# NeLy-EPFL/DeepFly3D

Hardware: AMD Instinct MI355X
Metric: frames/sec (7-view 2D->3D) (higher is better)
Workload: dtype f32; 1 GPU; BASELINE configs[1]: 2176 frames x 7 views 256x512x3 per GPU, 2-stack hourglass fp32, arg-max + 38-joint layout + fp64 DLT; frames_per_gpu=2176, parallelism=frame-sharded x1, one packed gather, collective_executed=False

## Files before the change

### deepfly3d_amd/csrc/hg_launch.h

```cpp
#pragma once
#include "hg_plan.h"

namespace {

inline int cu_count() {
    static int cached[64] = {0};
    int dev = 0;
    if (hipGetDevice(&dev) != hipSuccess || dev < 0 || dev >= 64) return 256;
    if (cached[dev] == 0) {
        int n = 0;
        cached[dev] = hipDeviceGetAttribute(&n, hipDeviceAttributeMultiprocessorCount, dev) == hipSuccess && n > 0 ? n : 256;
    }
    return cached[dev];
}

inline bool first_use_on_this_device(unsigned& mask) {
    int dev = 0;
    if (hipGetDevice(&dev) != hipSuccess || dev < 0 || dev > 31) return true;
    const bool first = !(mask & (1u << dev));
    mask |= 1u << dev;
    return first;
}

hipEvent_t get_event(df3d_hg* h) {
// ... 15 lines not shown
    ScopedTimer(df3d_hg* h_, hipStream_t s_, const std::string& name, const Work& w) : h(h_), s(s_), on(h_->prof.profiling) {
        if (!on) return;
        t = {get_event(h), get_event(h), h->prof.kernel_class(name), w};
        if (w.flops_executed < 0.0) t.w.flops_executed = w.flops;
        (void)hipEventRecord(t.a, s);
    }
    ~ScopedTimer() {
        if (!on) return;
        (void)hipEventRecord(t.b, s);
        h->prof.timed.push_back(t);
    }
};

template <typename T> struct TypeName;
template <> struct TypeName<float> { static constexpr const char* value = "float"; };
template <> struct TypeName<__hip_bfloat16> { static constexpr const char* value = "__hip_bfloat16"; };
template <> struct TypeName<_Float16> { static constexpr const char* value = "_Float16"; };
template <> struct TypeName<F32S> { static constexpr const char* value = "hgk::F32S"; };
template <typename T> using StorageT = std::conditional_t<std::is_same<T, F32S>::value, float, T>;

inline std::string targ(bool v) { return v ? "true" : "false"; }
inline std::string targ(int v) { return std::to_string(v); }
inline std::string targ(const char* v) { return v; }
template <typename... A>
std::string kname(const char* kernel, A... args) {
    std::string s = kernel;
    const char* sep = "<";
    ((s += sep, s += targ(args), sep = ", "), ...);
    return sizeof...(A) ? s + ">" : s;
}

template <auto KERNEL, typename... A>
int launch_kernel(df3d_hg* h, const std::string& name, const Work& w, dim3 grid, int threads, int lds_bytes, hipStream_t s, const A&... args) {
    ScopedTimer tm(h, s, name, w);
    static unsigned attr_done = 0;
    if (lds_bytes > 0 && first_use_on_this_device(attr_done))
        DF3D_HIP(hipFuncSetAttribute(reinterpret_cast<const void*>(KERNEL), hipFuncAttributeMaxDynamicSharedMemorySize, lds_bytes));
    hipLaunchKernelGGL(KERNEL, grid, dim3(threads), lds_bytes, s, args...);
    DF3D_LAUNCH_CHECK();
    return DF3D_OK;
}

template <typename T, int TAPS, int BN, int RB>
int launch_conv_t(df3d_hg* h, const ConvArgs& a, const Work& w, hipStream_t s) {
    const dim3 grid((unsigned)((a.M + BM - 1) / BM), (unsigned)(a.cout / BN));
    return launch_kernel<conv_mfma_kernel<T, TAPS, BN, RB>>(h, kname("conv_mfma_kernel", TypeName<T>::value, TAPS, BN, RB), w, grid, 256,
                                                            2 * (BM + BN) * (RB + 16), s, a);
}

template <typename T, int TAPS, int BN>
int launch_conv_rb(df3d_hg* h, const ConvArgs& a, int rb, const Work& w, hipStream_t s) {
    if (rb == 128) return launch_conv_t<T, TAPS, BN, 128>(h, a, w, s);
    return launch_conv_t<T, TAPS, BN, 64>(h, a, w, s);
}

template <typename T>
int launch_conv(df3d_hg* h, const ConvArgs& a, int taps, int rb, const Work& w, hipStream_t s) {
    int bn = (a.cout % 128 == 0) ? 128 : (a.cout % 64 == 0 ? 64 : 32);
    const long long wgs128 = ((a.M + BM - 1) / BM) * (a.cout / bn);
    if (bn == 128 && wgs128 < 2LL * cu_count()) bn = taps == 1 ? 32 : 64;
    if (taps == 1) {
        if (bn == 128) return launch_conv_rb<T, 1, 128>(h, a, rb, w, s);
        if (bn == 64) return launch_conv_rb<T, 1, 64>(h, a, rb, w, s);
        return launch_conv_rb<T, 1, 32>(h, a, rb, w, s);
    }
    if (bn == 128) return launch_conv_rb<T, 9, 128>(h, a, rb, w, s);
    if (bn == 64) return launch_conv_rb<T, 9, 64>(h, a, rb, w, s);
    df3d::set_error("3x3 convolution with cout %d unsupported", a.cout);
    return DF3D_EINVAL;
}

template <typename T, bool LAST>
int launch_head(df3d_hg* h, const HeadArgs& a, const Work& w, hipStream_t s) {
    return launch_kernel<head_kernel<T, LAST>>(h, kname("head_kernel", TypeName<T>::value, LAST), w, dim3((unsigned)((a.M + 127) / 128)), 256,
                                               HeadCfg<T, LAST>::LDS_BYTES, s, a);
}

struct BtLaunch {
    double px, m1;
    int tiles;
    bool pool_only;
};
inline double bt_flops(double px, int cin, int pl, bool conv1, bool ds, double taps3 = 9.0) {
    return 2.0 * px * ((conv1 ? (double)cin * pl : 0.0) + taps3 * pl * pl + 2.0 * pl * pl + (ds ? 2.0 * cin * pl : 0.0));
}
inline double bt_bytes(double px, int eb, int cin, int pl, bool t1, bool pool_only) {
    return px * eb * (cin + (t1 ? pl : 0) + (pool_only ? 0.5 * pl : 2.0 * pl));
}

template <typename T, int CIN, int PL, bool DS, bool UP = false, bool ADD2 = false>
int launch_bottleneck_t(df3d_hg* h, const BottleneckArgs& a, const BtLaunch& b, hipStream_t s) {
    return launch_kernel<bottleneck_kernel<T, CIN, PL, DS, UP, ADD2>>(
        h, kname("bottleneck_kernel", TypeName<T>::value, CIN, PL, DS, UP, ADD2),
        Work{bt_flops(b.px, CIN, PL, true, DS), bt_bytes(b.px, sizeof(T), CIN, PL, false, false), b.m1}, dim3(b.tiles), 256,
        BtCfg<T, CIN, PL, DS>::LDS_BYTES, s, a);
}

template <typename F>
int with_up_add2(const void* in2, const void* add2, F&& f) {
    if (in2) return f(std::true_type{}, std::false_type{});
    if (add2) return f(std::false_type{}, std::true_type{});
    return f(std::false_type{}, std::false_type{});
}

template <typename T>
int launch_l1_lp(df3d_hg* h, const BtL1Args& a, const BtLaunch& b, hipStream_t s) {
    const int tiles = a.V * (a.H / L1_TH) * (a.W / BT_TW);
    return launch_kernel<bottleneck_l1_kernel<T>>(h, kname("bottleneck_l1_kernel", TypeName<T>::value),
                                                  Work{bt_flops(b.px, 64, 64, true, true), bt_bytes(b.px, sizeof(T), 64, 64, false, b.pool_only), b.m1},
                                                  dim3(std::min(tiles, cu_count())), L1_WAVES * 64, L1_LDS_BYTES, s, a);
}

template <typename T, bool UP, int CIN, bool ADD2, int MODE>
int launch_ring_lp_(df3d_hg* h, const BtRingArgs& r, const BtLaunch& b, int lds_bytes, hipStream_t s) {
    return launch_kernel<bottleneck_ring_kernel<T, UP, CIN, ADD2, MODE>>(
        h, kname("bottleneck_ring_kernel", TypeName<T>::value, UP, CIN, ADD2, MODE),
        Work{bt_flops(b.px, CIN, 128, true, CIN == 128), bt_bytes(b.px, sizeof(T), CIN, 128, false, false), b.m1}, dim3(b.tiles), 256, lds_bytes, s, r);
}
template <typename T, bool UP, int CIN, bool ADD2 = false>
int launch_ring_lp(df3d_hg* h, const BtRingArgs& r, const BtLaunch& b, int lds_bytes, hipStream_t s) {
    return !r.w2d    ? launch_ring_lp_<T, UP, CIN, ADD2, 0>(h, r, b, lds_bytes, s)
           : h->ring2 ? launch_ring_lp_<T, UP, CIN, ADD2, 2>(h, r, b, lds_bytes, s)
                      : launch_ring_lp_<T, UP, CIN, ADD2, 1>(h, r, b, lds_bytes, s);
}

template <typename T, bool UP, bool ADD2, bool TAIL>
int launch_ring_f32(df3d_hg* h, const BtRingArgs& r, const BtLaunch& b, int lds_bytes, hipStream_t s) {
    return launch_kernel<bottleneck_ring_f32_kernel<UP, ADD2, TAIL, T>>(
        h, kname("bottleneck_ring_f32_kernel", UP, ADD2, TAIL, TypeName<T>::value),
        Work{bt_flops(b.px, 256, 128, !TAIL, false), bt_bytes(b.px, 4, 256, 128, TAIL, false), b.m1}, dim3(b.tiles), 256, lds_bytes, s, r);
}

inline int ring_lds_bytes() {
    int lds_bytes = BR_LDS_BYTES;
#ifdef DF3D_BT_TIMING
    if (const char* e = getenv("BR_LDS")) lds_bytes = atoi(e);
#endif
#ifdef BR_FORCE_LDS
    lds_bytes = BR_FORCE_LDS;
#endif
    return lds_bytes;
}

template <typename T, bool UP, int CIN, int PL>
int launch_conv1_f32(df3d_hg* h, const Conv1Args& c, const BtLaunch& b, hipStream_t s) {
    return launch_kernel<conv1_ring_f32_kernel<UP, CIN, PL, T>>(h, kname("conv1_ring_f32_kernel", UP, CIN, PL, TypeName<T>::value),
                                                                Work{2.0 * b.px * CIN * PL, b.px * 4.0 * (CIN + PL), 0.0},
                                                                dim3((unsigned)std::min<long long>(c.M / 128, 2LL * cu_count())), 256, C1_LDS_BYTES, s, c);
}

inline int launch_conv1_res_f32(df3d_hg* h, const Conv1Args& c, const BtLaunch& b, hipStream_t s) {
    return launch_kernel<conv1_res_f32_kernel>(h, kname("conv1_res_f32_kernel"), Work{2.0 * b.px * 256 * 128, b.px * 4.0 * (256 + 128), 0.0},
                                               dim3((unsigned)std::min<long long>(c.M / 128, (long long)(cu_count() & ~7))), 256, C1R_LDS_BYTES, s, c);
}

template <typename T>
int launch_layer1_tail_f32(df3d_hg* h, const BtRingArgs& r, const BtLaunch& b, hipStream_t s) {
    return launch_kernel<layer1_tail_f32_kernel<T>>(h, kname("layer1_tail_f32_kernel", TypeName<T>::value),
                                                    Work{bt_flops(b.px, 64, 64, false, true), bt_bytes(b.px, 4, 64, 64, true, b.pool_only), b.m1},
                                                    dim3(b.tiles), 256, L1F_LDS_BYTES, s, r);
}

template <typename T>
int launch_layer2_tail_f32(df3d_hg* h, const BtRingArgs& r, const BtLaunch& b, hipStream_t s) {
    return launch_kernel<layer2_tail_f32_kernel<T>>(h, kname("layer2_tail_f32_kernel", TypeName<T>::value),
                                                    Work{bt_flops(b.px, 128, 128, false, true), bt_bytes(b.px, 4, 128, 128, true, false), b.m1},
                                                    dim3(b.tiles), 256, L2F_LDS_BYTES, s, r);
}

template <bool UP, bool ADD2, bool L2>
int launch_wino_f32(df3d_hg* h, const BtRingArgs& r, const BtLaunch& b, hipStream_t s) {
    constexpr int CIN = L2 ? 128 : 256;
    const int cus = cu_count() & ~7;
    return launch_kernel<bottleneck_wino_f32_kernel<UP, ADD2, L2>>(
        h, kname("bottleneck_wino_f32_kernel", UP, ADD2, L2),
        Work{bt_flops(b.px, CIN, 128, false, L2), bt_bytes(b.px, 4, CIN, 128, true, false), b.m1, bt_flops(b.px, CIN, 128, false, L2, 3.0)},
        dim3(b.tiles <= cus ? b.tiles : cus), 256, WN_LDS_BYTES, s, r);
}

inline int launch_layer1_wino_f32(df3d_hg* h, const BtRingArgs& r, const BtLaunch& b, hipStream_t s) {
    const int tiles = r.V * (r.H / BT_TH) * (r.W / L1W_TW), cus = cu_count() & ~7;
    return launch_kernel<layer1_wino_f32_kernel>(
        h, kname("layer1_wino_f32_kernel"),
        Work{bt_flops(b.px, 64, 64, false, true), bt_bytes(b.px, 4, 64, 64, true, b.pool_only), b.m1, bt_flops(b.px, 64, 64, false, true, 4.0)},
        dim3(tiles <= cus ? tiles : cus), 256, L1W_LDS_BYTES, s, r);
}

template <typename T>
struct StepRun {
    static constexpr int eb = sizeof(T);
    df3d_hg* h;
    const float* images;
    float* heatmaps;
    unsigned char* act;
    int n_all, v0, n;
    hipStream_t s;
    const unsigned char* weights(size_t off) const {
        return reinterpret_cast<const unsigned char*>(std::is_same<T, float>::value ? (const void*)h->blob : h->lowp) + off * eb;
    }
    const unsigned char* wstream(long long off) const { return reinterpret_cast<const unsigned char*>(h->lowp) + h->stream_base() + off; }
    unsigned char* tptr(int id) const {
        if (id < 0) return nullptr;
        const TensorDesc& t = h->tensors[id];
        return act + (t.off * (size_t)n_all + (size_t)v0 * t.h * t.w * t.pitch) * eb;
    }
    double m1(const Step& st) const { return st.m1_elems * n * eb; }
};

template <typename T>
int launch_stem_step(const StepRun<T>& c, const Step& st) {
    constexpr int eb = sizeof(T);
    df3d_hg* const h = c.h;
    StemArgs a;
    a.img = c.images;
    a.out = c.tptr(st.out);
    a.w = h->blob + st.conv.w_off;
    a.w_lp = std::is_same<T, float>::value ? nullptr : c.weights(st.conv.w_off);
    a.bias = h->blob + st.conv.b_off;
    a.V = c.n;
    a.H = h->H;
    a.W = h->W;
    a.u8 = h->u8in;
    if (a.u8.frames) {
        a.u8.frames += (size_t)c.v0 * a.u8.FH * a.u8.FW * a.u8.FC;
        if (a.u8.flip) a.u8.flip += c.v0;
    }
    const int blocks = c.n * (h->H / 2 / STEM_TH) * (h->W / 2 / STEM_TW);
    const double opx = (double)c.n * (h->H / 2) * (h->W / 2);
    const Work w{2.0 * opx * 147 * 64, opx * (12.0 * 4 + 64.0 * eb), c.m1(st)};
    if constexpr (eb == 2) {
        return launch_kernel<stem_lp_kernel<T>>(h, kname("stem_lp_kernel", TypeName<T>::value), w, dim3(std::min(blocks, STEM_LP_WGS_PER_CU * cu_count())), 256, 0, c.s, a);
    } else if constexpr (std::is_same<T, F32S>::value) {
        return launch_kernel<stem_f32s_kernel>(h, kname("stem_f32s_kernel"), w, dim3(std::min(blocks, STEM_F32S_WGS_PER_CU * cu_count())), 256, 0, c.s, a);
    } else {
        return launch_kernel<stem_kernel<T>>(h, kname("stem_kernel", TypeName<T>::value), w, dim3(std::min(blocks, STEM_F32_WGS_PER_CU * cu_count())), 256, 0, c.s, a);
    }
}

template <typename T>
int launch_conv_step(const StepRun<T>& c, const Step& st) {
    constexpr int eb = sizeof(T);
    df3d_hg* const h = c.h;
    const TensorDesc& ti = h->tensors[st.in];
    ConvArgs a;
    a.in = c.tptr(st.in);
    a.out = c.tptr(st.out);
    a.res = c.tptr(st.res);
    a.out_nchw = st.conv.nchw_out ? c.heatmaps : nullptr;
    a.w = c.weights(st.conv.w_off);
    a.bias = h->blob + st.conv.b_off;
    a.scale = st.conv.preact ? h->blob + st.conv.s_off : nullptr;
    a.shift = st.conv.preact ? h->blob + st.conv.t_off : nullptr;
    a.M = (long long)c.n * ti.h * ti.w;
    a.H = ti.h;
    a.W = ti.w;
    a.cin = st.conv.cin_pad;
    a.cout = st.conv.cout_pad;
    a.in_pitch = ti.pitch;
    a.out_pitch = st.out >= 0 ? h->tensors[st.out].pitch : 0;
    a.res_pitch = st.res >= 0 ? h->tensors[st.res].pitch : 0;
    a.relu = st.conv.relu;
    a.cout_real = st.conv.cout;
    const int ke128 = 128 / eb;
    int rb = (st.conv.cin_pad % ke128 == 0) ? 128 : 64;
    if (h->rb_override == 64) rb = 64;
    const double mm = (double)a.M;
    const Work w{2.0 * mm * st.conv.taps * st.conv.cin * st.conv.cout, mm * eb * (st.conv.cin + st.conv.cout + (st.res >= 0 ? st.conv.cout : 0)), c.m1(st)};
    return launch_conv<T>(h, a, st.conv.taps, rb, w, c.s);
}

template <typename A>
void copy_block_args(A& a, const BtRingArgs& r) {
    a.in = r.in; a.out = r.out; a.pool = r.pool;
    a.b1 = r.b1; a.b2 = r.b2; a.b3 = r.b3; a.bd = r.bd; a.s1 = r.s1; a.t1 = r.t1;
    a.V = r.V; a.H = r.H; a.W = r.W;
}

template <typename T>
int launch_bottleneck_step(const StepRun<T>& c, const Step& st) {
    constexpr int eb = sizeof(T);
    constexpr bool F32 = std::is_same<T, float>::value;
    df3d_hg* const h = c.h;
    hipStream_t const s = c.s;
    const TensorDesc& ti = h->tensors[st.in];
    const bool ds = st.res < 0;
    const int cin = st.conv.cin, pl = st.conv.cout, n = c.n;
    const BtLaunch b{(double)n * ti.h * ti.w, c.m1(st), n * (ti.h / BT_TH) * (ti.w / BT_TW), st.pool_only};
    BtRingArgs r{};
    r.in = c.tptr(st.in);
    r.in2 = c.tptr(st.in2);
    r.add2 = c.tptr(st.add2);
    r.out = st.pool_only ? nullptr : c.tptr(st.out);
    r.pool = st.pool_only ? c.tptr(st.out) : c.tptr(st.pool_out);
    r.pool_in = c.tptr(st.pool_in);
    r.b1 = h->blob + st.conv.b_off;
    r.b2 = h->blob + st.conv2b.b_off;
    r.b3 = h->blob + st.conv3b.b_off;
    r.bd = ds ? h->blob + st.conv4b.b_off : nullptr;
    r.s1 = h->blob + st.conv.s_off;
    r.t1 = h->blob + st.conv.t_off;
    r.V = n;
    r.H = ti.h;
    r.W = ti.w;
    Conv1Args c1{};
    if (st.t1 >= 0) {
        c1.in = r.in;
        c1.in2 = r.in2;
        c1.H = ti.h;
        c1.W = ti.w;
        c1.t1 = c.tptr(st.t1);
        c1.wstream = c.wstream(st.wstream_c1);
        c1.b1 = r.b1;
        c1.s1 = r.s1;
        c1.t1c = r.t1;
        c1.M = (long long)n * ti.h * ti.w;
        r.t1in = c1.t1;
        r.zeros = c.wstream(h->zero_off);
        if (c1.M % 128) {
            df3d::set_error("conv1 of the split bottleneck needs whole 128-pixel tiles (M = %lld)", c1.M);
            return DF3D_EINVAL;
        }
    }
    switch (st.form) {
        case BT_REG: {
            BottleneckArgs a;
            copy_block_args(a, r);
            a.in2 = r.in2;
            a.add2 = r.add2;
            a.w1 = c.weights(st.conv.w_off);
            a.w2 = c.weights(st.conv2b.w_off);
            a.w3 = c.weights(st.conv3b.w_off);
            a.wd = ds ? c.weights(st.conv4b.w_off) : nullptr;
            if (cin == 256 && pl == 128)
                return with_up_add2(a.in2, a.add2, [&](auto up, auto add2) { return launch_bottleneck_t<T, 256, 128, false, up.value, add2.value>(h, a, b, s); });
            if (cin == 128 && pl == 128) return launch_bottleneck_t<T, 128, 128, true>(h, a, b, s);
            if (cin == 64 && pl == 64) return launch_bottleneck_t<T, 64, 64, true>(h, a, b, s);
            df3d::set_error("fused bottleneck %d -> %d unsupported", cin, pl);
            return DF3D_EINVAL;
        }
        case BT_L1_LP:
            if constexpr (eb == 2) {
                BtL1Args a;
                copy_block_args(a, r);
                a.wimage = c.wstream(st.wstream);
                return launch_l1_lp<T>(h, a, b, s);
            }
            break;
        case BT_RING_LP:
            if constexpr (eb == 2) {
                r.wstream = c.wstream(st.wstream);
                r.w2d = st.wstream_w2 >= 0 ? c.wstream(st.wstream_w2) : nullptr;
                if (cin == 128) return launch_ring_lp<T, false, 128>(h, r, b, BR_LDS_BYTES, s);
                return with_up_add2(r.in2, r.add2, [&](auto up, auto add2) { return launch_ring_lp<T, up.value, 256, add2.value>(h, r, b, ring_lds_bytes(), s); });
            }
            break;
        case BT_RING_F32:
            if constexpr (eb == 4) {
                r.wstream = c.wstream(st.wstream);
                return with_up_add2(r.in2, r.add2, [&](auto up, auto add2) { return launch_ring_f32<T, up.value, add2.value, false>(h, r, b, ring_lds_bytes(), s); });
            }
            break;
        case BT_SPLIT_F32:
            if constexpr (eb == 4) {
                if (int rc = r.in2 ? launch_conv1_f32<T, true, 256, 128>(h, c1, b, s) : launch_conv1_f32<T, false, 256, 128>(h, c1, b, s)) return rc;
                r.wstream = c.wstream(st.wstream);
                return with_up_add2(r.in2, r.add2, [&](auto up, auto add2) { return launch_ring_f32<T, up.value, add2.value, true>(h, r, b, ring_lds_bytes(), s); });
            }
            break;
        case BT_SPLIT_WINO:
            if constexpr (F32) {
                const bool resident = !r.in2 && h->c1res;
                if (resident) c1.wstream = c.wstream(st.wstream_wino + WN_STREAM_BYTES);
                if (int rc = resident   ? launch_conv1_res_f32(h, c1, b, s)
                             : r.in2 ? launch_conv1_f32<T, true, 256, 128>(h, c1, b, s)
                                     : launch_conv1_f32<T, false, 256, 128>(h, c1, b, s))
                    return rc;
                r.w2d = c.wstream(st.wstream_wino);
                r.wstream = c.wstream(st.wstream_u2);
                return with_up_add2(r.in2, r.add2, [&](auto up, auto add2) { return launch_wino_f32<up.value, add2.value, false>(h, r, b, s); });
            }
            break;
        case BT_L1F:
            if constexpr (eb == 4) {
                if (int rc = launch_conv1_f32<T, false, 64, 64>(h, c1, b, s)) return rc;
                r.wstream = c.wstream(st.wstream);
                return launch_layer1_tail_f32<T>(h, r, b, s);
            }
            break;
        case BT_L1F_WINO:
            if constexpr (F32) {
                if (int rc = launch_conv1_f32<T, false, 64, 64>(h, c1, b, s)) return rc;
                r.w2d = c.wstream(st.wstream_wino);
                return launch_layer1_wino_f32(h, r, b, s);
            }
            break;
        case BT_L2F:
            if constexpr (eb == 4) {
                if (int rc = launch_conv1_f32<T, false, 128, 128>(h, c1, b, s)) return rc;
                r.wstream = c.wstream(st.wstream);
                return launch_layer2_tail_f32<T>(h, r, b, s);
            }
            break;
        case BT_L2F_WINO:
            if constexpr (F32) {
                if (int rc = launch_conv1_f32<T, false, 128, 128>(h, c1, b, s)) return rc;
                r.w2d = c.wstream(st.wstream_wino);
                r.wstream = c.wstream(st.wstream_u2);
                return launch_wino_f32<false, false, true>(h, r, b, s);
            }
            break;
    }
    df3d::set_error("bottleneck form %d has no kernels for this element type", (int)st.form);
    return DF3D_EINVAL;
}

template <typename T>
int launch_head_step(const StepRun<T>& c, const Step& st) {
    constexpr int eb = sizeof(T);
    df3d_hg* const h = c.h;
    const TensorDesc& ti = h->tensors[st.in];
    HeadArgs a;
    a.r = c.tptr(st.in);
    a.x = st.last ? nullptr : c.tptr(st.res);
    a.out = st.last ? nullptr : c.tptr(st.out);
    a.heat = st.last ? c.heatmaps : nullptr;
    a.wfc = c.weights(st.conv.w_off);
    a.wsc = c.weights(st.conv2b.w_off);
    a.bfc = h->blob + st.conv.b_off;
    a.bsc = h->blob + st.conv2b.b_off;
    a.wfc_ = st.last ? nullptr : c.weights(st.conv3b.w_off);
    a.wsc_ = st.last ? nullptr : c.weights(st.conv4b.w_off);
    a.bfc_ = st.last ? nullptr : h->blob + st.conv3b.b_off;
    a.bsc_ = st.last ? nullptr : h->blob + st.conv4b.b_off;
    a.M = (long long)c.n * ti.h * ti.w;
    a.HW = ti.h * ti.w;
    a.fcstream = st.wstream >= 0 ? c.wstream(st.wstream) : nullptr;
    a.fc2stream = st.wstream2 >= 0 && a.M % 128 == 0 ? c.wstream(st.wstream2) : nullptr;
    const double mm = (double)a.M;
    const double fl = 2.0 * mm * (256.0 * 256 + 256.0 * 19 + (st.last ? 0.0 : 256.0 * 256 + 19.0 * 256));
    const Work w{fl, mm * eb * (st.last ? 256.0 : 768.0) + (st.last ? mm * 19 * 4 : 0.0), c.m1(st)};
    return st.last ? launch_head<T, true>(h, a, w, c.s) : launch_head<T, false>(h, a, w, c.s);
}

template <typename T>
int launch_pool_step(const StepRun<T>& c, const Step& st) {
    const TensorDesc& to = c.h->tensors[st.out];
    const int chunks = to.pitch * c.eb / 16;
    const long long total = (long long)c.n * to.h * to.w * chunks;
    return launch_kernel<pool2_kernel<StorageT<T>>>(c.h, kname("pool2_kernel", TypeName<StorageT<T>>::value), Work{0.0, (double)total * 16 * 5, c.m1(st)},
                                                    dim3((unsigned)((total + 255) / 256)), 256, 0, c.s, reinterpret_cast<const u32x4*>(c.tptr(st.in)),
                                                    reinterpret_cast<u32x4*>(c.tptr(st.out)), total, to.h, to.w, chunks);
}

template <typename T>
int launch_upadd_step(const StepRun<T>& c, const Step& st) {
    const TensorDesc& to = c.h->tensors[st.out];
    const int chunks = to.pitch * c.eb / 16;
    const long long total = (long long)c.n * to.h * to.w * chunks;
    return launch_kernel<upadd_kernel<StorageT<T>>>(c.h, kname("upadd_kernel", TypeName<StorageT<T>>::value), Work{0.0, (double)total * 16 * 2.25, c.m1(st)},
                                                    dim3((unsigned)((total + 255) / 256)), 256, 0, c.s, reinterpret_cast<const u32x4*>(c.tptr(st.in)),
                                                    reinterpret_cast<const u32x4*>(c.tptr(st.res)), reinterpret_cast<u32x4*>(c.tptr(st.out)), total, to.h,
                                                    to.w, chunks);
}

template <typename T>
int run_steps(df3d_hg* h, const float* images_all, int n_all, int upto, float* heatmaps_all, unsigned char* act, hipStream_t s) {
    auto launch = [&](int i, int v0, int n) -> int {
        const StepRun<T> c{h, images_all ? images_all + (size_t)v0 * h->H * h->W * 3 : nullptr,
                           heatmaps_all ? heatmaps_all + (size_t)v0 * h->classes * (h->H / 4) * (h->W / 4) : nullptr, act, n_all, v0, n, s};
        const Step& st = h->steps[i];
        switch (st.kind) {
            case ST_STEM: return launch_stem_step(c, st);
            case ST_CONV: return launch_conv_step(c, st);
            case ST_BOTTLENECK: return launch_bottleneck_step(c, st);
            case ST_HEAD: return launch_head_step(c, st);
            case ST_POOL: return launch_pool_step(c, st);
            case ST_UPADD: return launch_upadd_step(c, st);
        }
        return DF3D_OK;
    };
    for (int i = 0; i < upto;) {
        int j = i + 1;
        const int cv = h->chain_views;
        if (cv > 0 && cv < n_all && h->chain_end[i] > i + 1) {
            j = std::min(h->chain_end[i], upto);
            for (int v0 = 0; v0 < n_all; v0 += cv)
                for (int k = i; k < j; ++k)
                    if (int rc = launch(k, v0, std::min(cv, n_all - v0))) return rc;
        } else if (int rc = launch(i, 0, n_all)) {
            return rc;
        }
        i = j;
    }
    return DF3D_OK;
}

template <typename F>
auto with_elem_type(int dtype, F&& f) {
    switch (dtype) {
        case DF3D_DTYPE_F32: return f(float{});
        case DF3D_DTYPE_F32S: return f(F32S{});
        case DF3D_DTYPE_F16: return f(_Float16{});
        default: return f(__hip_bfloat16{});
    }
}

int run_steps_dtype(df3d_hg* h, const float* images, int n, int upto, float* heatmaps, unsigned char* act, hipStream_t s) {
    return with_elem_type(h->dtype, [&](auto t) { return run_steps<decltype(t)>(h, images, n, upto, heatmaps, act, s); });
}

}
```

### deepfly3d_amd/csrc/hg_plan.h

```cpp
#pragma once
#include <algorithm>
#include <string>
#include <vector>

#include "common.h"
#include "hg_types.h"
#include "hg_conv.h"
#include "hg_stem.h"
#include "hg_pool.h"
#include "hg_bt_reg.h"
#include "hg_bt_ring.h"
#include "hg_bt_l1.h"
#include "hg_head.h"
#include "hg_bt_ring_f32.h"
#include "hg_c1_f32.h"
#include "hg_l1_f32.h"
#include "hg_bt_wino_f32.h"
#include "hg_l1_wino_f32.h"
#include "hg_c1_res_f32.h"

using namespace hgk;

namespace {

enum StepKind { ST_STEM, ST_CONV, ST_POOL, ST_UPADD, ST_BOTTLENECK, ST_HEAD };

enum BtForm {
    BT_REG,
    BT_L1_LP,
    BT_RING_LP,
    BT_RING_F32,
    BT_SPLIT_F32,
    BT_SPLIT_WINO,
    BT_L1F,
    BT_L1F_WINO,
    BT_L2F,
    BT_L2F_WINO,
};

struct TensorDesc {
    size_t off;
    int h, w, c, pitch;
};

constexpr size_t VIRTUAL_OFF = ~size_t(0);

constexpr size_t L1F_WINO_UNUSED_SLOT_BYTES = L1F_STREAM_BYTES;

struct ConvPlan {
    int taps, cin, cout, cin_pad, cout_pad;
    bool preact, relu, nchw_out;
    size_t w_off, b_off, s_off, t_off;
};

struct Step {
    StepKind kind;
    std::string name;
    int in, out, res;
    ConvPlan conv;
    ConvPlan conv2b, conv3b, conv4b;
    bool last = false;
    int pool_out = -1;
    int in2 = -1;
    int add2 = -1;
    BtForm form = BT_REG;
    int pool_in = -1;
    bool pool_only = false;
    double m1_elems = 0;
    int t1 = -1;
    long long wstream = -1;
    long long wstream2 = -1;
    long long wstream_w2 = -1;
    long long wstream_c1 = -1;
    long long wstream_wino = -1;
    long long wstream_u2 = -1;
    int chain = -1;
};

struct Allocator {
    struct Blk { size_t off, size; };
    std::vector<Blk> free_list;
    size_t top = 0, peak = 0;
    size_t alloc(size_t n) {
        n = (n + 63) & ~size_t(63);
        for (size_t i = 0; i < free_list.size(); ++i)
            if (free_list[i].size >= n) {
                size_t off = free_list[i].off;
                free_list[i].off += n;
                free_list[i].size -= n;
                if (!free_list[i].size) free_list.erase(free_list.begin() + i);
                return off;
            }
        size_t off = top;
        top += n;
        peak = std::max(peak, top);
        return off;
    }
    void release(size_t off, size_t n) {
        n = (n + 63) & ~size_t(63);
        free_list.push_back({off, n});
        std::sort(free_list.begin(), free_list.end(), [](const Blk& a, const Blk& b) { return a.off < b.off; });
        for (size_t i = 0; i + 1 < free_list.size();) {
            if (free_list[i].off + free_list[i].size == free_list[i + 1].off) {
                free_list[i].size += free_list[i + 1].size;
                free_list.erase(free_list.begin() + i + 1);
            } else
                ++i;
        }
        if (!free_list.empty() && free_list.back().off + free_list.back().size == top) {
            top = free_list.back().off;
            free_list.pop_back();
        }
    }
};

struct Work {
    double flops, bytes, bytes_m1, flops_executed = -1.0;
};

struct HgProfile {
    bool profiling = false;
    struct Timed { hipEvent_t a, b; int cls; Work w; };
    std::vector<std::string> kernel_names;
    int kernel_class(const std::string& name) {
        for (size_t i = 0; i < kernel_names.size(); ++i)
            if (kernel_names[i] == name) return (int)i;
        kernel_names.push_back(name);
        return (int)kernel_names.size() - 1;
    }
    std::vector<Timed> timed;
    std::vector<hipEvent_t> event_pool;
};

}

struct df3d_hg {
    int dtype = DF3D_DTYPE_F32;
    int num_stacks = 2;
    int H = 256, W = 512;
    int classes = 19;
    int rb_override = 0;
    int fuse = 1;
    int fuse_upadd = 1;
    int l1 = 1;
    int ring = 1;
    int w2d = 1;
    int ring2 = 1;
    int split1 = 1;
    int wino = 1;
    int c1res = 1;
    bool split_id() const { return split1 == 1 || (split1 >= 8 && (split1 & 1)); }
    bool split_l1() const { return split1 == 1 || (split1 >= 8 && (split1 & 2)); }
    bool split_l2() const { return split1 == 1 || (split1 >= 8 && (split1 & 4)); }
    bool uses_zero_page = false;
    size_t zero_off = 0;
    int no_reuse = 0;
    int chain_views = 0;
    std::vector<int> chain_end;
    size_t stream_bytes = 0;
    hgk::StemU8 u8in{nullptr, nullptr, 0, 0, 0, {{0, 0, 0}, {1, 1, 1}, 0}};
    std::vector<TensorDesc> tensors;
    std::vector<int> pooled_of;
    std::vector<Step> steps;
    std::vector<df3d_hg_param> params;
    size_t blob_floats = 0;
    size_t act_elems_per_view = 0;
    const float* blob = nullptr;
    const void* lowp = nullptr;
    double flops_per_view = 0, elems_per_view = 0;

    Allocator alloc;
    HgProfile prof;

    bool lp() const { return dtype == DF3D_DTYPE_BF16 || dtype == DF3D_DTYPE_F16; }
    int elem_bytes() const { return lp() ? 2 : 4; }
    size_t stream_base() const { return lp() ? (blob_floats * 2 + 255) & ~size_t(255) : dtype == DF3D_DTYPE_F32S ? (blob_floats * 4 + 255) & ~size_t(255) : 0; }

    double m1_mark = 0;
    void m1_open() { m1_mark = elems_per_view; }
    void push_step(const Step& st) {
        steps.push_back(st);
        steps.back().chain = defer_frees ? plan_chain : -1;
    }
    void m1_close() { steps.back().m1_elems = elems_per_view - m1_mark; }
    static Step new_step(StepKind kind, const std::string& name, int in, int res) {
        Step st;
        st.kind = kind;
        st.name = name;
        st.in = in;
        st.res = res;
        return st;
    }
    int new_tensor(int h, int w, int c, int pitch = 0) {
        if (!pitch) pitch = c;
        TensorDesc t{alloc.alloc((size_t)h * w * pitch), h, w, c, pitch};
        tensors.push_back(t);
        pooled_of.push_back(-1);
        return (int)tensors.size() - 1;
    }
    int new_virtual_tensor(int h, int w, int c) {
        tensors.push_back(TensorDesc{VIRTUAL_OFF, h, w, c, c});
        pooled_of.push_back(-1);
        return (int)tensors.size() - 1;
    }
    bool defer_frees = false;
    int plan_chain = 0;
    std::vector<int> deferred;
    void free_tensor(int id) {
        if (defer_frees) {
            deferred.push_back(id);
            return;
        }
        const TensorDesc& t = tensors[id];
        if (no_reuse) return;
        if (t.off != VIRTUAL_OFF) alloc.release(t.off, (size_t)t.h * t.w * t.pitch);
    }
    void end_chain() {
        defer_frees = false;
        ++plan_chain;
        for (int id : deferred) free_tensor(id);
        deferred.clear();
    }
    long long take_stream(size_t bytes) {
        const long long off = (long long)stream_bytes;
        stream_bytes += bytes;
        return off;
    }
    size_t add_param(const std::string& name, int kind, int taps, int cin, int cout, int cin_pad, int cout_pad, size_t count,
                     int kperm = 0) {
        df3d_hg_param p;
        memset(&p, 0, sizeof(p));
        p.kperm = kperm;
        snprintf(p.name, sizeof(p.name), "%s", name.c_str());
        p.kind = kind;
        p.taps = taps;
        p.cin = cin;
        p.cout = cout;
        p.cin_pad = cin_pad;
        p.cout_pad = cout_pad;
        p.offset = blob_floats;
        p.count = count;
        blob_floats += (count + 63) & ~size_t(63);
        params.push_back(p);
        return p.offset;
    }

    ConvPlan plan_conv(const std::string& name, int taps, int cin, int cin_pad, int cout, bool preact, bool relu, bool nchw_out,
                       int kperm = 0) {
        const int cout_pad = (cout + 31) / 32 * 32;
        ConvPlan c{taps, cin, cout, cin_pad, cout_pad, preact, relu, nchw_out, 0, 0, 0, 0};
        c.w_off = add_param(name, 0, taps, cin, cout, cin_pad, cout_pad, (size_t)taps * cout_pad * cin_pad, kperm);
        c.b_off = add_param(name, 1, taps, cin, cout, cin_pad, cout_pad, cout_pad);
        if (preact) {
            c.s_off = add_param(name, 2, taps, cin, cout, cin_pad, cout_pad, cin_pad);
            c.t_off = add_param(name, 3, taps, cin, cout, cin_pad, cout_pad, cin_pad);
        }
        return c;
    }
    void account_conv(double px, int taps, int cin, int cout, bool res) {
        flops_per_view += 2.0 * px * taps * cin * cout;
        elems_per_view += px * (cin + cout + (res ? cout : 0));
    }
    int conv(const std::string& name, int in, int taps, int cout, bool preact, bool relu, int res, bool nchw_out = false) {
        const TensorDesc ti = tensors[in];
        Step st = new_step(ST_CONV, name, in, res);
        st.conv = plan_conv(name, taps, ti.c, ti.pitch, cout, preact, relu, nchw_out);
        st.out = nchw_out ? -1 : new_tensor(ti.h, ti.w, cout, st.conv.cout_pad);
        m1_open();
        push_step(st);
        account_conv((double)ti.h * ti.w, taps, ti.c, cout, res >= 0);
        m1_close();
        return st.out;
    }
    bool can_add2(int x) const {
        const TensorDesc& t = tensors[x];
        return fuse && t.c == 256 && t.h % 8 == 0 && t.w % 16 == 0;
    }
    int bottleneck(const std::string& name, int x, int planes, bool want_pool = false, int x2 = -1, bool only_pool = false, bool pool_input = false,
                   int a2 = -1, const std::string& sum_name = std::string()) {
        const int cin = tensors[x].c, cout = 2 * planes;
        const TensorDesc tx = tensors[x];
        const bool shape_ok = (cin == 256 && planes == 128) || (cin == 128 && planes == 128) || (cin == 64 && planes == 64);
        const bool fused_here = fuse && shape_ok && tx.h % 8 == 0 && tx.w % 16 == 0;
        if (x2 >= 0 && !(fused_here && fuse_upadd && cin == 256 && planes == 128)) {
            upadd(name + ".upadd", x, x2);
            x2 = -1;
        }
        if (fused_here) {
            const bool ds = cin != cout;
            m1_open();
            Step st;
            st.kind = ST_BOTTLENECK;
            st.name = name + ".conv3";
            st.in = x;
            st.in2 = x2;
            st.add2 = a2;
            if (a2 >= 0) st.name = sum_name;
            if (x2 >= 0 || a2 >= 0) elems_per_view += (double)tx.h * tx.w * cin * 2.25;
            st.res = ds ? -1 : x;
            st.conv = plan_conv(name + ".conv1", 1, cin, cin, planes, true, true, false);
            st.conv2b = plan_conv(name + ".conv2", 9, planes, planes, planes, false, true, false);
            if (ds) st.conv4b = plan_conv(name + ".downsample.0", 1, cin, cin, cout, false, false, false);
            st.conv3b = plan_conv(name + ".conv3", 1, planes, planes, cout, false, false, false, lp() ? 1 : 0);
// ... 259 lines not shown
```

### deepfly3d_amd/csrc/hourglass.hip

```cpp
#include "hg_plan.h"
#include "hg_launch.h"
#include "hg_weights.h"
static_assert(hgk::WN_U2_BYTES <= hgk::BRF_STREAM_BYTES, "U's second part fits the identity block's stage-image slot");
static_assert(hgk::WN_U2_BYTES <= hgk::L2F_STREAM_BYTES, "layer2: U's second part fits the stage-image slot");

namespace {

int check_forward_args(df3d_hg* h, const void* images, int n, void* ws, size_t ws_bytes) {
    DF3D_CHECK_ARG(h != nullptr, "null handle");
    if (!h->blob) {
        df3d::set_error("df3d_hg_forward: weights not set (call df3d_hg_set_weights first)");
        return DF3D_ESTATE;
    }
    DF3D_CHECK_ARG(n > 0, "n must be positive");
    DF3D_CHECK_ARG(images && ws, "null pointer");
    DF3D_CHECK_ARG(ws_bytes >= df3d_hg_workspace_bytes(h, n), "workspace too small");
    DF3D_CHECK_ARG((reinterpret_cast<uintptr_t>(ws) & 255) == 0, "workspace must be 256-byte aligned");
    return DF3D_OK;
}

}

extern "C" {

#ifdef DF3D_BT_TIMING
int df3d_dbg_ring_cycles(unsigned long long* out8) {
    if (hipMemcpyFromSymbol(out8, HIP_SYMBOL(hgk::br_dbg), 96) != hipSuccess) return -1;
    unsigned long long z[12] = {0, 0, 0, 0, 0, 0, 0, 0, 0, 0, 0, 0};
    return hipMemcpyToSymbol(HIP_SYMBOL(hgk::br_dbg), z, 96) == hipSuccess ? 0 : -1;
}
#endif

int df3d_hg_create(int dtype, int num_stacks, df3d_hg** out) {
    DF3D_CHECK_ARG(out != nullptr, "null out");
    DF3D_CHECK_ARG(dtype == DF3D_DTYPE_F32 || dtype == DF3D_DTYPE_BF16 || dtype == DF3D_DTYPE_F16 || dtype == DF3D_DTYPE_F32S, "dtype must be DF3D_DTYPE_F32, DF3D_DTYPE_BF16, DF3D_DTYPE_F16 or DF3D_DTYPE_F32S");
    DF3D_CHECK_ARG(num_stacks >= 1 && num_stacks <= 8, "num_stacks must be in [1, 8]");
    df3d_hg* h = new df3d_hg();
    h->dtype = dtype;
    h->num_stacks = num_stacks;
    h->build();
    *out = h;
    return DF3D_OK;
}

void df3d_hg_destroy(df3d_hg* h) {
    if (!h) return;
    for (auto& t : h->prof.timed) {
        (void)hipEventDestroy(t.a);
        (void)hipEventDestroy(t.b);
    }
    for (auto e : h->prof.event_pool) (void)hipEventDestroy(e);
    delete h;
}

int df3d_hg_set_input(df3d_hg* h, int height, int width) {
    DF3D_CHECK_ARG(h != nullptr, "null handle");
    DF3D_CHECK_ARG(height > 0 && width > 0 && height % 64 == 0 && width % 64 == 0, "input height and width must be multiples of 64");
    h->H = height;
    h->W = width;
    h->build();
    return DF3D_OK;
}

int df3d_hg_set_option(df3d_hg* h, const char* key, int value) {
    struct Option {
        const char* key;
        int df3d_hg::*member;
        bool (*accepts)(int value);
        const char* bad_value;
        bool replans;
        const char* after_weights;
        bool on_off = false;
    };
    constexpr auto bit = [](int v) { return v == 0 || v == 1; };
    static const Option options[] = {
        {"fuse", &df3d_hg::fuse, bit, "fuse must be 0 or 1", true, "set 'fuse' before df3d_hg_set_weights (it changes the parameter manifest)"},
        {"fuse_upadd", &df3d_hg::fuse_upadd, [](int v) { return v >= 0 && v <= 2; }, "fuse_upadd must be 0, 1 or 2", true,
         "set 'fuse_upadd' before df3d_hg_set_weights (it changes the plan)"},
        {"l1", &df3d_hg::l1, bit, "l1 must be 0 or 1", true, "set 'l1' before df3d_hg_set_weights (it changes the plan and the low-precision buffer)"},
        {"ring", &df3d_hg::ring, bit, "ring must be 0 or 1", true, "set 'ring' before df3d_hg_set_weights (it changes the low-precision buffer)"},
        {"w2d", &df3d_hg::w2d, bit, "w2d must be 0 or 1", true, "set 'w2d' before df3d_hg_set_weights (it changes the weight streams)"},
        {"ring2", &df3d_hg::ring2, bit, "ring2 must be 0 or 1", false, nullptr},
        {"split1", &df3d_hg::split1, [](int v) { return v == 0 || v == 1 || (v >= 8 && v < 16); },
         "split1 must be 0, 1 or 8 + a mask (1 identity blocks, 2 layer1, 4 layer2)", true,
         "set 'split1' before df3d_hg_set_weights (it changes the plan and the weight streams)"},
        {"wino", &df3d_hg::wino, bit, "wino must be 0 or 1", true, "set 'wino' before df3d_hg_set_weights (it changes the weight streams)"},
        {"c1res", &df3d_hg::c1res, bit, "c1res must be 0 or 1", false, nullptr},
        {"no_reuse", &df3d_hg::no_reuse, bit, "no_reuse must be 0 or 1", true, "set 'no_reuse' before df3d_hg_set_weights (it changes the workspace plan)"},
        {"chain_views", &df3d_hg::chain_views, [](int v) { return v >= 0; }, "chain_views must be >= 0", true,
         "switch 'chain_views' on or off before df3d_hg_set_weights (it changes the workspace plan)", true},
        {"row_bytes", &df3d_hg::rb_override, [](int v) { return v == 0 || v == 64 || v == 128; }, "row_bytes must be 0, 64 or 128", false, nullptr},
    };
    DF3D_CHECK_ARG(h && key, "null argument");
    for (const Option& o : options) {
        if (strcmp(key, o.key)) continue;
        DF3D_CHECK_ARG(o.accepts(value), o.bad_value);
        const bool replan = o.replans && (!o.on_off || (value > 0) != (h->*o.member > 0));
        DF3D_CHECK_ARG(!replan || h->blob == nullptr, o.after_weights);
        h->*o.member = value;
        if (replan) h->build();
        return DF3D_OK;
    }
    df3d::set_error("df3d_hg_set_option: unknown key %s", key);
    return DF3D_EINVAL;
}

int df3d_hg_num_params(const df3d_hg* h) { return h ? (int)h->params.size() : 0; }

int df3d_hg_param_desc(const df3d_hg* h, int i, df3d_hg_param* out) {
    DF3D_CHECK_ARG(h && out, "null argument");
    DF3D_CHECK_ARG(i >= 0 && i < (int)h->params.size(), "index out of range");
    *out = h->params[i];
    return DF3D_OK;
}

size_t df3d_hg_blob_floats(const df3d_hg* h) { return h ? h->blob_floats : 0; }

size_t df3d_hg_lowp_bytes(const df3d_hg* h) {
    if (!h) return 0;
    return h->stream_base() + h->stream_bytes;
}

int df3d_hg_set_weights(df3d_hg* h, const float* blob_dev, void* lowp_dev, void* stream) {
    return hg_weights::df3d_hg_set_weights(h, blob_dev, lowp_dev, df3d::as_stream(stream));
}

size_t df3d_hg_workspace_bytes(const df3d_hg* h, int n) {
    if (!h || n <= 0) return 0;
    return h->act_elems_per_view * (size_t)n * h->elem_bytes() + 256;
}

int df3d_hg_forward(df3d_hg* h, const float* images_dev, int n, float* heatmaps_dev, void* workspace_dev,
                    size_t workspace_bytes, void* stream) {
    if (int rc = check_forward_args(h, images_dev, n, workspace_dev, workspace_bytes)) return rc;
    DF3D_CHECK_ARG(heatmaps_dev != nullptr, "null heatmaps");
    unsigned char* act = reinterpret_cast<unsigned char*>(workspace_dev);
    return run_steps_dtype(h, images_dev, n, (int)h->steps.size(), heatmaps_dev, act, df3d::as_stream(stream));
}

int df3d_hg_forward_u8(df3d_hg* h, const unsigned char* frames_dev, const unsigned char* flip_dev, int n, int frame_h, int frame_w, int frame_c,
                       const float* mean3_host, const float* std3_host, int resize, float* heatmaps_dev, void* workspace_dev, size_t workspace_bytes,
                       void* stream) {
    if (int rc = check_forward_args(h, frames_dev, n, workspace_dev, workspace_bytes)) return rc;
    DF3D_CHECK_ARG(heatmaps_dev != nullptr && mean3_host && std3_host, "null pointer");
    DF3D_CHECK_ARG(frame_h > 0 && frame_w > 0 && (frame_c == 1 || frame_c == 3), "bad frame shape (C must be 1 or 3)");
    DF3D_CHECK_ARG(resize >= DF3D_RESIZE_BILINEAR && resize <= DF3D_RESIZE_AREA, "resize must be one of DF3D_RESIZE_*");
    hgk::StemU8 u;
    u.nm.resize = resize;
    u.frames = frames_dev;
    u.flip = flip_dev;
    u.FH = frame_h;
    u.FW = frame_w;
    u.FC = frame_c;
    for (int c = 0; c < 3; ++c) {
        DF3D_CHECK_ARG(std3_host[c] != 0.0f, "std must be non-zero");
        u.nm.mean[c] = mean3_host[c];
        u.nm.inv_std[c] = 1.0f / std3_host[c];
    }
    h->u8in = u;
    unsigned char* act = reinterpret_cast<unsigned char*>(workspace_dev);
    const int rc = run_steps_dtype(h, nullptr, n, (int)h->steps.size(), heatmaps_dev, act, df3d::as_stream(stream));
    h->u8in.frames = nullptr;
    return rc;
}

int df3d_hg_work(const df3d_hg* h, int n, double* flops, double* bytes) {
    DF3D_CHECK_ARG(h && flops && bytes, "null argument");
    *flops = h->flops_per_view * n;
    *bytes = h->elems_per_view * n * h->elem_bytes();
    return DF3D_OK;
}

int df3d_hg_profile(df3d_hg* h, int enable) {
    DF3D_CHECK_ARG(h != nullptr, "null handle");
    h->prof.profiling = enable != 0;
    for (auto& t : h->prof.timed) {
        h->prof.event_pool.push_back(t.a);
        h->prof.event_pool.push_back(t.b);
    }
    h->prof.timed.clear();
    return DF3D_OK;
}

int df3d_hg_profile_count(const df3d_hg* h) { return h ? (int)h->prof.kernel_names.size() : 0; }

int df3d_hg_profile_read(df3d_hg* h, int kernel_class, char* name_buf, int buflen, double* ms, double* flops, double* bytes, double* bytes_m1,
                         int* launches) {
    DF3D_CHECK_ARG(h && name_buf && buflen > 0 && ms && flops && bytes && bytes_m1 && launches, "null argument");
    DF3D_CHECK_ARG(kernel_class >= 0 && kernel_class < (int)h->prof.kernel_names.size(), "kernel_class out of range");
    snprintf(name_buf, buflen, "%s", h->prof.kernel_names[kernel_class].c_str());
    *ms = *flops = *bytes = *bytes_m1 = 0.0;
    *launches = 0;
    for (auto& t : h->prof.timed) {
        if (t.cls != kernel_class) continue;
        DF3D_HIP(hipEventSynchronize(t.b));
        float e = 0.f;
        DF3D_HIP(hipEventElapsedTime(&e, t.a, t.b));
        *ms += e;
        *flops += t.w.flops;
        *bytes += t.w.bytes;
        *bytes_m1 += t.w.bytes_m1;
        *launches += 1;
    }
    return DF3D_OK;
}

int df3d_hg_profile_executed_flops(df3d_hg* h, int kernel_class, double* flops_executed) {
    DF3D_CHECK_ARG(h && flops_executed, "null argument");
    DF3D_CHECK_ARG(kernel_class >= 0 && kernel_class < (int)h->prof.kernel_names.size(), "kernel_class out of range");
    *flops_executed = 0.0;
    for (auto& t : h->prof.timed)
        if (t.cls == kernel_class) *flops_executed += t.w.flops_executed;
    return DF3D_OK;
}

int df3d_hg_num_steps(const df3d_hg* h) { return h ? (int)h->steps.size() : 0; }

double df3d_hg_step_m1_bytes(const df3d_hg* h, int step, int n) {
    if (!h || step < 0 || step >= (int)h->steps.size() || n <= 0) return 0.0;
    return h->steps[step].m1_elems * n * h->elem_bytes();
}

int df3d_hg_step_desc(const df3d_hg* h, int step, char* name_buf, int buflen, int* hwc) {
    DF3D_CHECK_ARG(h && name_buf && hwc && buflen > 0, "null argument");
    DF3D_CHECK_ARG(step >= 0 && step < (int)h->steps.size(), "step out of range");
    const Step& st = h->steps[step];
    snprintf(name_buf, buflen, "%s", st.name.c_str());
    if (st.out >= 0) {
        const TensorDesc& t = h->tensors[st.out];
        hwc[0] = t.h;
        hwc[1] = t.w;
        hwc[2] = t.c;
    } else {
        hwc[0] = h->H / 4;
        hwc[1] = h->W / 4;
        hwc[2] = h->classes;
    }
    return DF3D_OK;
}

// ... 24 lines not shown
```

Before: 752.9 frames/s.

## Add weight-resident persistent conv1 kernel for upsample-add and layer2 bottlenecks

Adds a persistent 1x1-conv kernel that keeps the full conv1 weights resident in LDS, double-buffers input tiles across a grid-stride loop, and fuses the upsample-add and BN+ReLU before the MFMA multiply. It is used for split-Winograd bottlenecks whose input carries an upsampled second operand, and for layer2 Winograd blocks, in place of the ring-streamed conv1. It also adds an option to switch it off. The aim is to stop re-streaming weights for every tile and to overlap loads with compute. In exchange it runs one workgroup per CU because of the large LDS footprint, and the upsample path depends on W%32 and H%2 shape conditions.

Result: no change. 756.4 frames/s (median of 6 runs) (+0.5%).

```diff
diff --git a/deepfly3d_amd/csrc/hg_c1_resx_f32.h b/deepfly3d_amd/csrc/hg_c1_resx_f32.h
--- /dev/null
+++ b/deepfly3d_amd/csrc/hg_c1_resx_f32.h
@@ -0,0 +1,221 @@
+#pragma once
+#include <type_traits>
+
+#include "hg_bt_common.h"
+#include "hg_bt_wino_f32.h"
+#include "hg_c1_f32.h"
+#include "hg_types.h"
+
+namespace hgk {
+
+#ifndef C1RX_ABL
+#define C1RX_ABL 0
+#endif
+
+constexpr int c1rx_lds_bytes(int cin) { return (cin / 16) * BR_STAGE_BYTES + 512 * 4 + 128 * 4; }
+static_assert(c1rx_lds_bytes(256) <= 160 * 1024, "one workgroup per CU");
+
+__device__ __forceinline__ f32x2 c1rx_pk_add(f32x2 a, f32x2 b) {
+    f32x2 r;
+    asm("v_pk_add_f32 %0, %1, %2" : "=v"(r) : "v"(a), "v"(b));
+    return r;
+}
+
+template <bool UP, int CIN, int PL>
+__global__ __launch_bounds__(256, 1) void conv1_resx_f32_kernel(Conv1Args p) {
+    static_assert(PL == 128 && ((UP && CIN == 256) || (!UP && CIN == 128)), "instantiated shapes");
+    constexpr int NST = CIN / 16;
+    constexpr int NQ = CIN / 8;
+    constexpr int NP = NQ / 8;
+    constexpr int LP = UP ? 16 : 8;
+    constexpr int NS = (C1RX_ABL & 4) ? 0 : 16;
+    constexpr int W_BYTES = NST * BR_STAGE_BYTES;
+    extern __shared__ __attribute__((aligned(16))) unsigned char smem[];
+    float* const coef_lds = reinterpret_cast<float*>(smem + W_BYTES);
+
+    const int tid = threadIdx.x, lane = tid & 63;
+    const int wave = __builtin_amdgcn_readfirstlane(tid >> 6);
+    const int half = lane >> 5, l31 = lane & 31;
+    {
+        if constexpr (UP) {
+            const unsigned w_addr = lds_addr(smem);
+            const unsigned wvoff = (unsigned)wave * 2048u + (unsigned)lane * 16u;
+#pragma unroll
+            for (int k = 0; k < NST; ++k) br_ring_issue(p.wstream, k, w_addr + (unsigned)(k * BR_STAGE_BYTES), wave, wvoff);
+        } else {
+            const unsigned char* const ws = reinterpret_cast<const unsigned char*>(p.wstream);
+#pragma unroll
+            for (int k = 0; k < NST * 2; ++k) {
+                const int idx = k * 256 + tid, s = idx >> 9, rem = idx & 511, c = rem & 3, r = rem >> 2;
+                const int ch = 4 * (r & 31) + (r >> 5);
+                *reinterpret_cast<u32x4*>(smem + s * BR_STAGE_BYTES + br_swz(r, c)) = *reinterpret_cast<const u32x4*>(ws + s * BR_STAGE_BYTES + br_swz(ch, c));
+            }
+        }
+        if (tid < CIN) {
+            coef_lds[tid] = p.s1[tid];
+            coef_lds[256 + tid] = p.t1c[tid];
+        }
+        if (tid < 128) coef_lds[512 + tid] = p.b1[tid];
+        asm volatile("s_waitcnt vmcnt(0)" ::: "memory");
+        br_barrier();
+    }
+    const long long ntiles = p.M / 32, stride = 4LL * gridDim.x;
+    long long t = 4LL * blockIdx.x + wave;
+    if (t >= ntiles) return;
+
+    const unsigned char* const wf0 = smem + br_swz(l31, half);
+    const unsigned char* const wf1 = smem + br_swz(l31, 2 + half);
+    const unsigned xlane = (unsigned)((l31 * CIN + 4 * half) * 4);
+    const unsigned ylane = (unsigned)((l31 >> 1) * 1024 + 16 * half);
+    const unsigned olane = (unsigned)(((4 * half) * 128 + 4 * l31) * 4);
+    const float* const cs_l = coef_lds + 4 * half;
+    const unsigned char* const in = reinterpret_cast<const unsigned char*>(p.in);
+    const unsigned char* const in2 = reinterpret_cast<const unsigned char*>(p.in2);
+    unsigned char* const out = reinterpret_cast<unsigned char*>(p.t1);
+
+    const int tpr = UP ? p.W / 32 : 1;
+    const int s_rows = UP ? (int)(stride / tpr) : 0, s_pieces = UP ? (int)(stride - (long long)s_rows * tpr) : 0;
+    int R = UP ? (int)(t / tpr) : 0, xt = UP ? (int)(t - (long long)R * tpr) : 0;
+    auto y_of = [&](int row, int piece) { return in2 + ((size_t)(row >> 1) * (size_t)(p.W / 2) + (size_t)(16 * piece)) * 1024; };
+
+    f32x4 xs[2][2][4];
+    f32x4 ys[UP ? 2 : 1][2][4];
+    auto issue_part = [&](auto B, long long tile, const unsigned char* ybase, int part) {
+        constexpr int b = decltype(B)::value;
+        const unsigned char* const sb = in + (size_t)tile * (32 * CIN * 4) + part * 256;
+#pragma unroll
+        for (int m = 0; m < 2; ++m) {
+            if (C1RX_ABL & 2) asm volatile("" : "+v"(xs[b][m][0]), "+v"(xs[b][m][1]), "+v"(xs[b][m][2]), "+v"(xs[b][m][3]));
+            else wn_xload4s<32>(xs[b][m], sb + m * 128, xlane);
+        }
+        if constexpr (UP) {
+#pragma unroll
+            for (int m = 0; m < 2; ++m) {
+                if (C1RX_ABL & 2) asm volatile("" : "+v"(ys[b][m][0]), "+v"(ys[b][m][1]), "+v"(ys[b][m][2]), "+v"(ys[b][m][3]));
+                else wn_xload4s<32>(ys[b][m], ybase + part * 256 + m * 128, ylane);
+            }
+        }
+    };
+    auto wait_part = [&](auto B, auto N) {
+        constexpr int b = decltype(B)::value;
+        if (C1RX_ABL & 2) return;
+#pragma unroll
+        for (int m = 0; m < 2; ++m) wn_uwait<decltype(N)::value>(xs[b][m]);
+        if constexpr (UP) {
+#pragma unroll
+            for (int m = 0; m < 2; ++m) wn_uwait<decltype(N)::value>(ys[b][m]);
+        }
+    };
+    auto bn_relu = [&](f32x4 (&x)[4], const f32x4 (&y)[4], int q0) {
+        if (C1RX_ABL & 1) return;
+#pragma unroll
+        for (int j = 0; j < 4; ++j) {
+            const f32x4 cs = *reinterpret_cast<const f32x4*>(cs_l + 8 * (q0 + j));
+            const f32x4 ct = *reinterpret_cast<const f32x4*>(cs_l + 256 + 8 * (q0 + j));
+            f32x4 v = x[j];
+            if constexpr (UP) {
+                const f32x2 lo = c1rx_pk_add(f32x2{x[j][0], x[j][1]}, f32x2{y[j][0], y[j][1]}), hi = c1rx_pk_add(f32x2{x[j][2], x[j][3]}, f32x2{y[j][2], y[j][3]});
+                v = f32x4{lo[0], lo[1], hi[0], hi[1]};
+            }
+#pragma unroll
+            for (int e = 0; e < 4; ++e) x[j][e] = br_relu(fmaf(v[e], cs[e], ct[e]));
+        }
+    };
+    f32x16 o[4];
+    f32x4 wfq[2];
+    auto wf_of = [&](int n) {
+        const int q = (n >> 2) & (NQ - 1), i = n & 3;
+        return *reinterpret_cast<const f32x4*>(((q & 1) ? wf1 : wf0) + (q >> 1) * BR_STAGE_BYTES + i * 2048);
+    };
+    auto multiply = [&](const f32x4 (&x)[4], int q0) {
+#pragma unroll
+        for (int j = 0; j < 4; ++j)
+#pragma unroll
+            for (int i = 0; i < 4; ++i) {
+                const int n = 4 * (q0 + j) + i;
+                wfq[(n + 1) & 1] = wf_of(n + 1);
+                __builtin_amdgcn_sched_barrier(0);
+                if (C1RX_ABL & 8) o[i][0] += x[j][0] * wfq[n & 1][0];
+                else mfma_quad<float>(x[j][0], x[j][1], x[j][2], x[j][3], wfq[n & 1], o[i]);
+                __builtin_amdgcn_sched_barrier(0);
+            }
+    };
+    wfq[0] = wf_of(0);
+
+    using B0 = std::integral_constant<int, 0>;
+    using B1 = std::integral_constant<int, 1>;
+    const unsigned char* yt = UP ? y_of(R, xt) : nullptr;
+    const unsigned char* yn = yt;
+    issue_part(B0{}, t, yt, 0);
+    issue_part(B1{}, t, yt, 1);
+    bool first = true;
+    long long tn = t;
+    auto part = [&](auto PT) {
+        constexpr int pt = decltype(PT)::value;
+        using B = std::integral_constant<int, pt & 1>;
+        if constexpr (pt == 0) {
+            if (first && !(C1RX_ABL & 2)) asm volatile("s_waitcnt vmcnt(%0)" ::"n"(LP) : "memory");
+            wait_part(B{}, std::integral_constant<int, LP + NS>{});
+        } else {
+            wait_part(B{}, std::integral_constant<int, LP>{});
+        }
+#pragma unroll
+        for (int m = 0; m < 2; ++m) {
+            bn_relu(xs[pt & 1][m], ys[UP ? (pt & 1) : 0][m], 8 * pt + 4 * m);
+            __builtin_amdgcn_sched_barrier(0);
+            multiply(xs[pt & 1][m], 8 * pt + 4 * m);
+            __builtin_amdgcn_sched_barrier(0);
+        }
+        if constexpr (pt == NP - 1) {
+            unsigned char* const ot = out + (size_t)t * (32 * 512);
+#pragma unroll
+            for (int r = 0; r < 16; ++r) {
+                const f32x4 v = {br_relu(o[0][r]), br_relu(o[1][r]), br_relu(o[2][r]), br_relu(o[3][r])};
+                if (!(C1RX_ABL & 4) || v[0] == 12345.678f) *reinterpret_cast<f32x4*>(ot + ((r & 3) + 8 * (r >> 2)) * 512 + olane) = v;
+            }
+            __builtin_amdgcn_sched_barrier(0);
+        }
+        if constexpr (pt + 2 < NP) issue_part(B{}, t, yt, pt + 2);
+        else issue_part(B{}, tn, yn, pt + 2 - NP);
+        __builtin_amdgcn_sched_barrier(0);
+    };
+#pragma unroll 1
+    for (;;) {
+        tn = t;
+        int Rn = R, xn = xt;
+        if (t + stride < ntiles) {
+            tn = t + stride;
+            if constexpr (UP) {
+                Rn = R + s_rows;
+                xn = xt + s_pieces;
+                if (xn >= tpr) {
+                    xn -= tpr;
+                    ++Rn;
+                }
+            }
+        }
+        if constexpr (UP) yn = y_of(Rn, xn);
+#pragma unroll
+        for (int i = 0; i < 4; ++i) {
+            const float bias = coef_lds[512 + 4 * l31 + i];
+#pragma unroll
+            for (int r = 0; r < 16; ++r) o[i][r] = bias;
+        }
+        part(std::integral_constant<int, 0>{});
+        part(std::integral_constant<int, 1>{});
+        if constexpr (NP == 4) {
+            part(std::integral_constant<int, 2>{});
+            part(std::integral_constant<int, 3>{});
+        }
+        if (tn == t) break;
+        t = tn;
+        R = Rn;
+        xt = xn;
+        yt = yn;
+        first = false;
+    }
+    wait_part(B0{}, std::integral_constant<int, 0>{});
+    wait_part(B1{}, std::integral_constant<int, 0>{});
+}
+
+}
diff --git a/deepfly3d_amd/csrc/hg_launch.h b/deepfly3d_amd/csrc/hg_launch.h
--- a/deepfly3d_amd/csrc/hg_launch.h
+++ b/deepfly3d_amd/csrc/hg_launch.h
@@ -191,6 +191,15 @@
 inline int launch_conv1_res_f32(df3d_hg* h, const Conv1Args& c, const BtLaunch& b, hipStream_t s) {
     return launch_kernel<conv1_res_f32_kernel>(h, kname("conv1_res_f32_kernel"), Work{2.0 * b.px * 256 * 128, b.px * 4.0 * (256 + 128), 0.0},
                                                dim3((unsigned)std::min<long long>(c.M / 128, (long long)(cu_count() & ~7))), 256, C1R_LDS_BYTES, s, c);
+}
+
+inline bool c1resx_takes(const Conv1Args& c) { return c.W % 32 == 0 && c.H % 2 == 0; }
+template <bool UP, int CIN>
+int launch_conv1_resx_f32(df3d_hg* h, const Conv1Args& c, const BtLaunch& b, hipStream_t s) {
+    return launch_kernel<conv1_resx_f32_kernel<UP, CIN, 128>>(h, kname("conv1_resx_f32_kernel", UP, CIN, 128),
+                                                              Work{2.0 * b.px * CIN * 128, b.px * 4.0 * (CIN + 128), 0.0},
+                                                              dim3((unsigned)std::min<long long>(c.M / 128, (long long)(cu_count() & ~7))), 256,
+                                                              c1rx_lds_bytes(CIN), s, c);
 }
 
 template <typename T>
@@ -408,9 +417,9 @@
             break;
         case BT_SPLIT_WINO:
             if constexpr (F32) {
-                const bool resident = !r.in2 && h->c1res;
+                const bool resident = r.in2 ? h->c1resx && c1resx_takes(c1) : h->c1res != 0;
                 if (resident) c1.wstream = c.wstream(st.wstream_wino + WN_STREAM_BYTES);
-                if (int rc = resident   ? launch_conv1_res_f32(h, c1, b, s)
+                if (int rc = resident   ? (r.in2 ? launch_conv1_resx_f32<true, 256>(h, c1, b, s) : launch_conv1_res_f32(h, c1, b, s))
                              : r.in2 ? launch_conv1_f32<T, true, 256, 128>(h, c1, b, s)
                                      : launch_conv1_f32<T, false, 256, 128>(h, c1, b, s))
                     return rc;
@@ -442,7 +451,7 @@
             break;
         case BT_L2F_WINO:
             if constexpr (F32) {
-                if (int rc = launch_conv1_f32<T, false, 128, 128>(h, c1, b, s)) return rc;
+                if (int rc = h->c1resx ? launch_conv1_resx_f32<false, 128>(h, c1, b, s) : launch_conv1_f32<T, false, 128, 128>(h, c1, b, s)) return rc;
                 r.w2d = c.wstream(st.wstream_wino);
                 r.wstream = c.wstream(st.wstream_u2);
                 return launch_wino_f32<false, false, true>(h, r, b, s);
diff --git a/deepfly3d_amd/csrc/hg_plan.h b/deepfly3d_amd/csrc/hg_plan.h
--- a/deepfly3d_amd/csrc/hg_plan.h
+++ b/deepfly3d_amd/csrc/hg_plan.h
@@ -18,6 +18,7 @@
 #include "hg_bt_wino_f32.h"
 #include "hg_l1_wino_f32.h"
 #include "hg_c1_res_f32.h"
+#include "hg_c1_resx_f32.h"
 
 using namespace hgk;
 
@@ -149,6 +150,7 @@
     int split1 = 1;
     int wino = 1;
     int c1res = 1;
+    int c1resx = 1;
     bool split_id() const { return split1 == 1 || (split1 >= 8 && (split1 & 1)); }
     bool split_l1() const { return split1 == 1 || (split1 >= 8 && (split1 & 2)); }
     bool split_l2() const { return split1 == 1 || (split1 >= 8 && (split1 & 4)); }
diff --git a/deepfly3d_amd/csrc/hourglass.hip b/deepfly3d_amd/csrc/hourglass.hip
--- a/deepfly3d_amd/csrc/hourglass.hip
+++ b/deepfly3d_amd/csrc/hourglass.hip
@@ -86,6 +86,7 @@
          "set 'split1' before df3d_hg_set_weights (it changes the plan and the weight streams)"},
         {"wino", &df3d_hg::wino, bit, "wino must be 0 or 1", true, "set 'wino' before df3d_hg_set_weights (it changes the weight streams)"},
         {"c1res", &df3d_hg::c1res, bit, "c1res must be 0 or 1", false, nullptr},
+        {"c1resx", &df3d_hg::c1resx, bit, "c1resx must be 0 or 1", false, nullptr},
         {"no_reuse", &df3d_hg::no_reuse, bit, "no_reuse must be 0 or 1", true, "set 'no_reuse' before df3d_hg_set_weights (it changes the workspace plan)"},
         {"chain_views", &df3d_hg::chain_views, [](int v) { return v >= 0; }, "chain_views must be >= 0", true,
          "switch 'chain_views' on or off before df3d_hg_set_weights (it changes the workspace plan)", true},
```
